# d3sm0/gym_pomdp

Measured on AMD Instinct MI355X. Metric: env steps/sec (whole node), RockSample(7,8) batch=2^20, 1/2/4/8 MI355X, higher is better.
Workload: dtype int32

## Files before the change

gym_pomdp_amd/csrc/envs/rock.hip.h:

```cpp
#pragma once
#include "../envs_common.hip.h"

namespace pomdp {

template <int W, bool STOCH = false>
struct RockEnv {
    using Params = pomdp_rock_params;
    using Reward = int32_t;
    using S = typename std::conditional<W == 1, uint32_t, uint64_t>::type;
    static constexpr int WORDS = W;
    static constexpr const char *NAME = STOCH ? (W == 1 ? "StochasticRockEnv<1>" : "StochasticRockEnv<2>") : (W == 1 ? "RockEnv<1>" : "RockEnv<2>");
    static constexpr bool POOLED_LPT2 = !STOCH;
    static constexpr bool QUAD_STEP = true;
    static constexpr bool HAS_ROCKS = true;
    static constexpr bool POOLED_ANY_LPT = !STOCH;
    static constexpr bool STOCHASTIC = STOCH;
    static constexpr bool QUAD_TAB = true;
    struct Shared {
        uint2 thr[32];
        int8_t grid[256];
        uint8_t rxy[16];
        uint16_t rpos[16];
        uint32_t dir_y[16];
        uint32_t dir_x[16];
// ... 43 lines not shown
        sh.dir_x[tid] = left | (right << 16);
        sh.row[tid] = same;
    }

    static __device__ __forceinline__ void load(State &st, const uint32_t *state, int64_t n, uint32_t i)
    {
        st.s = ld_stream(state + i);
        if (W == 2) st.s |= (S)((uint64_t)ld_stream(state + n + i) << 32);
    }
    static __device__ __forceinline__ void store(const State &st, uint32_t *state, int64_t n, uint32_t i, bool)
    {
        st_stream(state + i, (uint32_t)st.s);
        if (W == 2) st_stream(state + n + i, (uint32_t)((uint64_t)st.s >> 32));
    }

    static __device__ __forceinline__ uint32_t elem(const uint4 &w, uint32_t e) { return e == 0 ? w.x : e == 1 ? w.y : e == 2 ? w.z : w.w; }

    template <class LowWord>
    static __device__ __forceinline__ bool k53_le(uint32_t H, uint32_t th, uint32_t tl, LowWord lo)
    {
        const uint32_t kh = H >> 5;
        bool r = kh < th;
        if (kh == th) r = (lo() >> 6) <= tl;
        return r;
    }
    static __device__ __forceinline__ uint32_t rock_code_hi(uint32_t H)
    {
        const uint32_t kh = H >> 5;
        return kh > HALF_HI ? 2u : (kh < HALF_HI ? 0u : 3u);
    }
    static __device__ __forceinline__ uint32_t rock_code_lo(uint32_t L) { return (L >> 6) ? 2u : 1u; }
    template <bool AUTO = false>
    static __device__ __forceinline__ uint4 reset_block(const RngKey &key, uint32_t lane, uint32_t j2)
    {
        const uint32_t c3 = AUTO ? (((uint32_t)POMDP_STREAM_STEP << 24) | (SENSOR_BLOCK + j2)) : (((uint32_t)POMDP_STREAM_RESET << 24) | j2);
        return philox4x32_10(lane >> 2, key.t_lo, key.t_hi, c3, key.k0, key.k1);
    }
    template <bool AUTO>
    static __device__ __forceinline__ uint32_t reset_codes(const RngKey &key, uint32_t lane, int K)
    {
        return reset_codes<AUTO>(elem(reset_block<AUTO>(key, lane, 0u), lane & 3u), key, lane, K);
    }
    template <bool AUTO>
    static __device__ __forceinline__ uint32_t reset_codes(uint32_t w, const RngKey &key, uint32_t lane, int K)
    {
        uint32_t codes = w & 0xAAAAAAAAu;
        if (__popc(w) <= 6) reset_ties<AUTO>(w, key, lane, K, codes, 0);
        return codes & (K >= 16 ? 0xFFFFFFFFu : ((1u << (2 * K)) - 1u));
    }
    template <bool AUTO>
    static __device__ __forceinline__ void reset_ties(uint32_t w, const RngKey &key, uint32_t lane, int K, uint32_t &word, int base)
    {
        bool have_lo = false;
        uint32_t l = 0;
        for (int j = 0; j < K; ++j) {
            const uint32_t rot = (uint32_t)(2 * j + 2) & 31u;
            if (rock_code_hi(__builtin_rotateright32(w, rot)) != 3u) continue;
            if (!have_lo) {
                uint32_t lane_ = lane;
                asm volatile("" : "+v"(lane_));
                l = elem(reset_block<AUTO>(rare_key(key), lane_, 1u), lane & 3u);
                have_lo = true;
            }
            const uint32_t c = rock_code_lo(__builtin_rotateright32(l, rot));
            word = (word & ~(3u << (base + 2 * j))) | (c << (base + 2 * j));
        }
    }
    static __device__ __forceinline__ uint4 quad_block(const RngKey &key, uint32_t lane, uint32_t j2)
    {
        return philox4x32_10(lane >> 2, key.t_lo, key.t_hi, ((uint32_t)POMDP_STREAM_STEP << 24) | j2, key.k0, key.k1);
    }

    static __device__ __forceinline__ void reset_codes4(const uint32_t (&R)[4], const RngKey &key, uint32_t first, int K,
                                                        uint32_t (&codes)[4])
    {
        const uint32_t exist = K >= 16 ? 0xFFFFFFFFu : ((1u << (2 * K)) - 1u);
#pragma unroll
        for (int e = 0; e < 4; ++e) codes[e] = R[e] & 0xAAAAAAAAu & exist;
        if (min(min(__popc(R[0]), __popc(R[1])), min(__popc(R[2]), __popc(R[3]))) <= 6) {
#pragma unroll
            for (int e = 0; e < 4; ++e) codes[e] = reset_codes<true>(R[e], key, first + (uint32_t)e, K);
        }
    }
    template <int N, bool ROT>
    static __device__ __forceinline__ void fresh_states(const uint32_t (&R)[N], const RngKey &key, uint32_t first, int K,
                                                        uint32_t start, uint32_t (&fresh)[N])
    {
        const uint32_t exist = K >= 16 ? 0xFFFFFFFFu : ((1u << (2 * K)) - 1u);
        auto word = [&](uint32_t codes) { return ROT ? (codes | start) : (start | (codes << 8)); };
        int fewest = __popc(R[0]);
#pragma unroll
        for (int e = 0; e < N; ++e) { fresh[e] = word(R[e] & (0xAAAAAAAAu & exist)); fewest = min(fewest, (int)__popc(R[e])); }
        if (fewest <= 6) {
#pragma unroll
            for (int e = 0; e < N; ++e)
                if (__popc(R[e]) <= 6) reset_ties<true>(R[e], key, first + (uint32_t)e, K, fresh[e], ROT ? 0 : 8);
        }
    }
    static __device__ __forceinline__ int reset(const Shared &, const Params &p, State &st, const RngKey &key,
                                                uint32_t lane)
    {
        const uint64_t s = (uint32_t)p.start_x | ((uint32_t)p.start_y << 4);
        st.s = (S)(s | ((uint64_t)reset_codes<false>(key, lane, p.num_rocks) << 8));
        return 0;
    }
    static __device__ __forceinline__ int reset_ob(const Params &, const State &) { return 0; }

    static __device__ __forceinline__ void reset_where(const Shared &, const Params &p, State &st, bool fresh,
                                                       const RngKey &key, uint32_t lane)
    {
        if (!__any(fresh)) return;
        const uint32_t codes = reset_codes<true>(key, lane, p.num_rocks);
        if (fresh) st.s = (S)((uint64_t)((uint32_t)p.start_x | ((uint32_t)p.start_y << 4)) | ((uint64_t)codes << 8));
    }
    static __device__ __forceinline__ void reset_where_chain(const Shared &sh, const Params &p, State &st, bool fresh,
                                                             const RngKey &key, uint32_t lane, const RngKey &akey,
                                                             uint32_t n_actions, int &next_action)
    {
        reset_where_chain_default<RockEnv>(sh, p, st, fresh, key, lane, akey, n_actions, next_action);
    }
    static __device__ __forceinline__ S fresh_state(const Params &p, uint32_t w, const RngKey &key, uint32_t lane)
    {
        return (S)((uint64_t)((uint32_t)p.start_x | ((uint32_t)p.start_y << 4)) | ((uint64_t)reset_codes<true>(w, key, lane, p.num_rocks) << 8));
    }

    static __device__ __forceinline__ int legal_count(const Shared &sh, const Params &p, const State &st, uint32_t &pre,
                                                      int &n_pre, uint32_t &alive)
    {
        const S s = st.s;
        const int x = (int)(s & 15u), y = (int)((s >> 4) & 15u), K = p.num_rocks;
        pre = 1u; n_pre = 1;
        if (y + 1 < p.size) { pre |= 0u << (3 * n_pre); ++n_pre; }
        if (y - 1 >= 0) { pre |= 2u << (3 * n_pre); ++n_pre; }
        if (x - 1 >= 0) { pre |= 3u << (3 * n_pre); ++n_pre; }
        const int id = sh.grid[x * 16 + y];
        if (id >= 0 && id < K && ((uint32_t)(s >> (8 + 2 * (id & 15))) & 3u) != 1u) { pre |= 4u << (3 * n_pre); ++n_pre; }
        const uint64_t r = (uint64_t)s >> 8;
        const uint64_t even = 0x5555555555555555ull;
        const uint64_t spread = ~(r & ~(r >> 1)) & even & ((1ull << (2 * K)) - 1ull);
        alive = (uint32_t)spread;
        return n_pre + __popc(alive);
    }
    struct Legal { uint32_t pre, alive; int n_pre, count; };
    static __device__ __forceinline__ Legal legal_set(const Shared &sh, const Params &p, const State &st)
    {
        Legal L;
        L.count = legal_count(sh, p, st, L.pre, L.n_pre, L.alive);
        return L;
    }
    static __device__ __forceinline__ int legal_pick(const Shared &sh, const Legal &L, int idx)
    {
        if (idx < L.n_pre) return (int)((L.pre >> (3 * idx)) & 7u);
        const int j = nth_set_bit<2>(L.alive, idx - L.n_pre) >> 1;
        const uint32_t rxy = sh.rxy[j & 15];
        return 5 + sh.grid[(rxy & 15u) * 16 + (rxy >> 4)];
    }
    static __device__ __forceinline__ int legal_nth(const Shared &sh, const Params &p, const State &st, int idx)
    {
        return legal_pick(sh, legal_set(sh, p, st), idx);
    }
    static __device__ __forceinline__ int legal_count(const Shared &sh, const Params &p, const State &st)
    {
        uint32_t pre, alive; int n_pre;
        return legal_count(sh, p, st, pre, n_pre, alive);
    }

    static __device__ __forceinline__ bool check_ok(int measured, int count, double pv)
    {
        return measured < 5 && abs(count) < 2 && 0 < pv && pv < 1;
    }
    static __device__ __forceinline__ void belief_update(const Shared &sh, const Params &p, const State &st, int a, int ob,
                                                         const pomdp_rock_belief &b, int64_t n, uint32_t i, uint32_t &ck)
    {
        const S s = st.s;
        const int x = (int)(s & 15u), y = (int)((s >> 4) & 15u), r = (a - 5) & 15;
        const uint32_t rxy = sh.rxy[r];
// ... 48 lines not shown
        const bool north = (am & dy & 0xFFFFu) != 0, south = (am & (dy >> 16)) != 0;
        const bool west = (same & dx & 0xFFFFu) != 0, east = (same & (dx >> 16)) != 0;
        uint32_t m = (alive & ck) << 5;
        if (y + 1 < p.size && north) m |= 1u << 0;
        if (east) m |= 1u << 1;
        if (y - 1 >= 0 && south) m |= 1u << 2;
        if (x - 1 >= 0 && west) m |= 1u << 3;
        return m;
    }

    static __device__ __forceinline__ int select_target(const Shared &sh, const Params &p, const State &st,
                                                        const pomdp_rock_belief &b, int64_t n, uint32_t i)
    {
        const S s = st.s;
        const int x = (int)(s & 15u), y = (int)((s >> 4) & 15u), K = p.num_rocks;
        int best = 4 * p.size * p.size, best_rock = -1;
        for (int j = 0; j < K; ++j) {
            if (((uint32_t)(s >> (8 + 2 * j)) & 3u) == 1u || b.count[(int64_t)j * n + i] < 0) continue;
            const uint32_t rxy = sh.rxy[j];
            const int dx = x - (int)(rxy & 15u), dy = y - (int)(rxy >> 4), d2 = dx * dx + dy * dy;
            if (d2 < best) { best = d2; best_rock = j; }
        }
        return best_rock;
    }

    static __device__ __forceinline__ double compute_prob(const Shared &sh, const Params &p, const State &st, int a, int ob)
    {
        if (a <= 4) return ob == 0 ? 1.0 : 0.0;
        const S s = st.s;
        const int x = (int)(s & 15u), y = (int)((s >> 4) & 15u), r = (a - 5) & 15;
        const uint32_t rxy = sh.rxy[r];
        const double eff = p.eff[abs(x - (int)(rxy & 15u)) + abs(y - (int)(rxy >> 4))];
        const uint32_t code = (uint32_t)(s >> (8 + 2 * r)) & 3u;
        if ((ob == 2 && code == 2u) || (ob == 1 && code == 0u)) return eff;
        return 1 - eff;
    }

    template <class RT>
    static __device__ __forceinline__ void step_pre(const Shared &sh, const Params &p, State &st, int a, RT &rew,
                                                    int &done, Aux &aux)
    {
        const S s = st.s;
        const uint32_t x = (uint32_t)s & 15u, y = ((uint32_t)s >> 4) & 15u;
        const uint32_t size = (uint32_t)p.size, K = (uint32_t)p.num_rocks;
        const int r = (a - 5) & 15;
        const uint32_t rp = sh.rpos[r];
        const uint32_t d = __builtin_amdgcn_sad_u8(x | (y << 8), rp, 0u);
        aux.th = sh.thr[d].x;
        aux.r = (uint8_t)r;
        aux.good = ((uint32_t)(s >> (8 + 2 * r)) & 3u) == 2u;
        aux.want = a > 4;
        const int penalty = STOCH ? 0 : -100;
        const int id = sh.grid[x * 16 + y];
        const int sh_ = 8 + 2 * (id & 15);
        const uint32_t code = (uint32_t)(s >> sh_) & 3u;
        const bool sample_ok = ((uint32_t)id < K) & (code != 1u);
        const uint32_t a2 = (uint32_t)a << 1;
        const uint32_t nx = x + (uint32_t)__builtin_amdgcn_sbfe(0xC4, a2, 2u), ny = y + (uint32_t)__builtin_amdgcn_sbfe(0x31, a2, 2u);
        const bool inside = max(nx, ny) < size;
        const bool is_move = a < 4, is_sample = a == 4, east = a == 1;
        const bool moved = is_move & inside, left = is_move & !inside, sampled = is_sample & sample_ok,
                   missed = is_sample & !sample_ok;
        const uint32_t d_move = ((uint32_t)s & 0xFFu) ^ (nx | (ny << 4));
        const S d_sample = (S)(code ^ 1u) << sh_;
        st.s = s ^ (moved ? (S)d_move : (sampled ? d_sample : (S)0));
        const bool good_rock = code == 2u;
        int rw = ((left & east) | (sampled & good_rock)) ? 10 : 0;
        rw = (sampled & !good_rock) ? -10 : rw;
        rw = ((left & !east) | missed) ? penalty : rw;
        rew = rw;
        if (STOCH) done = left & east;
        else done = left | missed;
    }
    static __device__ __forceinline__ uint32_t thr_lo_of(const Shared &sh, const State &st, int r)
    {
        const uint32_t x = (uint32_t)st.s & 15u, y = ((uint32_t)st.s >> 4) & 15u;
        return sh.thr[__builtin_amdgcn_sad_u8(x | (y << 8), sh.rpos[r & 15], 0u)].y;
    }
    static constexpr int TAB_ACTIONS = W == 1 ? 17 : 21;

    static constexpr uint32_t REC_LUT_LO = 0x0A0A9CF6u, REC_LUT_HI = 0x00000000u;
    using TabEntry = typename std::conditional<W == 1, uint2, uint32_t>::type;
    struct RecTab { TabEntry e[TAB_ACTIONS][256]; };
    static __device__ __forceinline__ uint32_t rec_f(uint32_t off, int c, uint32_t ob_mask, uint32_t oc)
    {
        const uint32_t rbyte = (((uint64_t)REC_LUT_HI << 32 | REC_LUT_LO) >> (8u * oc)) & 0xFFu;
        return off | (((uint32_t)c & 3u) << 5) | (ob_mask << 8) | (rbyte << 16) | ((oc & 1u) << 24);
    }
    static constexpr uint32_t ROT_POS = 24u;
    template <bool ROT = false>
    static __device__ __forceinline__ void build_rec_tab(RecTab &tab, const Shared &sh, const Params &p, int pos)
    {
        static_assert(!ROT || W == 1, "the rotated layout is the one-state-word loops'");
        constexpr uint32_t POS0 = ROT ? ROT_POS : 0u, ROCK0 = ROT ? 0u : 8u;
        const uint32_t x = (uint32_t)pos & 15u, y = (uint32_t)pos >> 4, size = (uint32_t)p.size, K = (uint32_t)p.num_rocks;
        const int id = sh.grid[x * 16 + y];
        const uint32_t NOTHING = 6u << 28, PENALTY = (STOCH ? 6u : 1u) << 28, EXIT_EAST = 3u << 28;
        const uint32_t NO_TIE = 1u << 27;
        for (int a = 0; a < 5 + (int)K && a < TAB_ACTIONS; ++a) {
            uint32_t e, f;
            if (a < 4) {
                const uint32_t nx = x + (uint32_t)((a == 1) - (a == 3)), ny = y + (uint32_t)((a == 0) - (a == 2));
                const bool inside = max(nx, ny) < size;
                e = inside ? (((uint32_t)pos ^ (nx | (ny << 4))) | NOTHING) : (a == 1 ? EXIT_EAST : PENALTY);
                e |= NO_TIE;
                f = rec_f(POS0 + ((a & 1) ? 0u : 4u), inside ? (a < 2 ? 1 : -1) : 0, 0u, e >> 28 & 7u);
            } else if (a == 4) {
                const bool rock = (uint32_t)id < K;
                e = (rock ? ((8u + 2u * (uint32_t)id) | 0x80000000u) : 0u) | PENALTY | NO_TIE;
                f = rec_f(rock ? ROCK0 + 2u * (uint32_t)id : 0u, 0, 0u, e >> 28 & 7u);
            } else {
                e = sh.thr[__builtin_amdgcn_sad_u8(x | (y << 8), sh.rpos[a - 5], 0u) & 31u].x | NOTHING;
                f = rec_f(ROCK0 + 2u * (uint32_t)(a - 5), 0, 3u, 6u);
            }
            if constexpr (W == 1) tab.e[a][pos] = make_uint2(e, f);
            else tab.e[a][pos] = e;
        }
    }
    template <bool ROT = false>
    static __device__ __forceinline__ uint2 rec_lookup(const RecTab &tab, uint32_t s, uint32_t a)
    {
        if constexpr (ROT) {
            const uint32_t off = __builtin_amdgcn_alignbit(a, s, ROT_POS - 3u) & ~7u;
            return *reinterpret_cast<const uint2 *>(reinterpret_cast<const char *>(&tab.e[0][0]) + off);
        } else return tab.e[a][s & 0xFFu];
    }
    static __device__ __forceinline__ uint32_t rec_kh(uint32_t H) { return __builtin_amdgcn_alignbit(12u, H, 5u); }
    template <bool ROT = false>
    static __device__ __forceinline__ uint32_t rec_thr_lo(const Shared &sh, uint32_t s, uint32_t a, uint32_t f)
    {
        if constexpr (ROT) return thr_lo_of(sh, State{(S)(s >> ROT_POS)}, (int)((f & 31u) >> 1));
        else return thr_lo_of(sh, State{(S)s}, (int)a - 5);
    }
    static __device__ __forceinline__ void rec_finish(const uint2 ef, uint32_t &s, uint32_t a, bool correct, uint32_t fresh, uint32_t &rec)
    {
        const uint32_t e = ef.x, f = ef.y;
        const uint32_t q = __builtin_amdgcn_ubfe(s, f, 2u);
        const bool ok = ((int32_t)e < 0) & (q != 1u);
        const uint32_t keep = ((q == 2u) == correct) ? 0xFFFFFE00u : 0xFFFFFD00u;
        const uint32_t rfb = (f & keep) | a;
        const uint32_t rok = 0x00F60004u - q * 0x00760000u;
        rec = ok ? rok : rfb;
        const int c = ok ? 1 - (int)q : __builtin_amdgcn_sbfe((int)f, 5u, 2u);
        const uint32_t moved = s + ((uint32_t)c << (f & 31u));
        s = rec >= (1u << 24) ? fresh : moved;
    }
    template <class LowWord>
    static __device__ __forceinline__ void step_rec(const Shared &sh, const RecTab &tab, S &s, uint32_t a, uint32_t H, S fresh,
                                                    uint32_t &rec, LowWord lo)
    {
        const uint32_t s_lo = (uint32_t)s, s_hi = W == 2 ? (uint32_t)((uint64_t)s >> 32) : 0u;
        if constexpr (W == 1) {
            const uint2 ef = rec_lookup(tab, s_lo, a);
            const uint32_t kh = rec_kh(H);
            bool correct = kh < ef.x;
            if (kh == ef.x) correct = (lo() >> 6) <= rec_thr_lo(sh, s_lo, a, ef.y);
            uint32_t sn = s_lo;
            rec_finish(ef, sn, a, correct, (uint32_t)fresh, rec);
            s = (S)sn;
        } else {
            const uint32_t e = tab.e[a][s_lo & 0xFFu];
            const bool up_s = (e & 32u) != 0u;
            const uint32_t code = __builtin_amdgcn_ubfe(up_s ? s_hi : s_lo, e, 2u);
            const bool ok = ((int32_t)e < 0) & (code != 1u);
            const uint32_t collect = (code ^ 1u) << (e & 31u);
            const uint32_t move = (a < 4u ? e : 0u) & 0xFFu;
            const uint32_t d_lo = (ok & !up_s) ? collect : move, d_hi = (ok & up_s) ? collect : 0u;
            const uint32_t oc = ok ? code : __builtin_amdgcn_ubfe(e, 28u, 3u);
            const uint32_t rbyte = __builtin_amdgcn_perm(REC_LUT_HI, REC_LUT_LO, (oc << 16) | 0x0C000C0Cu);
            const uint32_t done = oc & 1u;
            const uint32_t gi = 2u * a - 1u;
            const bool good = __builtin_amdgcn_ubfe((gi & 32u) ? s_hi : s_lo, gi, 1u) != 0u;
            const uint32_t kh = __builtin_amdgcn_alignbit(12u, H, 5u);
            bool correct = kh < e;
            if (a > 4u && kh == e) correct = (lo() >> 6) <= thr_lo_of(sh, State{s}, (int)a - 5);
            const uint32_t ob = a > 4u ? ((good == correct) ? 2u << 8 : 1u << 8) : 0u;
            rec = rbyte | (done << 24) | ob | a;
            s = done ? fresh : (S)(((uint64_t)(s_hi ^ d_hi) << 32) | (s_lo ^ d_lo));
        }
    }

    template <class LowWord>
    static __device__ __forceinline__ int sensor_ob(const Shared &sh, const State &st, const Aux &aux, uint32_t H, LowWord lo)
    {
        const uint32_t kh = H >> 5;
        bool correct = kh < aux.th;
        if (kh == aux.th) correct = (lo() >> 6) <= thr_lo_of(sh, st, aux.r);
        return aux.want ? ((aux.good == correct) ? 2 : 1) : 0;
    }

    static constexpr bool QUAD_SENSOR = !STOCH;
    template <class RT>
    static __device__ __forceinline__ void step_with_H(const Shared &sh, const Params &p, State &st, int a, const RngKey &key,
                                                       uint32_t lane, uint32_t H, int &ob, RT &rew, int &done)
    {
        Aux aux;
        step_pre(sh, p, st, a, rew, done, aux);
        ob = sensor_ob(sh, st, aux, H, [&]() { return elem(quad_block(key, lane, 1u), lane & 3u); });
    }

    template <class RT>
    static __device__ __forceinline__ void step(const Shared &sh, const Params &p, State &st, int a,
                                                const RngKey &key, uint32_t lane, int &ob, RT &rew, int &done)
    {
        const uint32_t e = lane & 3u;
        if (STOCH) {
            const uint4 g = quad_block(key, lane, 0u);
            const bool act = k53_le(elem(g, e), (uint32_t)(p.act_thr >> 26), (uint32_t)p.act_thr & LO_MASK,
                                    [&]() { return elem(quad_block(key, lane, 1u), e); }) != (p.act_gt != 0);
            State nx = st;
            Aux aux; RT r2; int d2;
            step_pre(sh, p, nx, a, r2, d2, aux);
            const uint4 h = quad_block(key, lane, 2u);
            const int o2 = sensor_ob(sh, nx, aux, elem(h, e), [&]() { return elem(quad_block(key, lane, 3u), e); });
            if (act) { st = nx; rew = r2; done = d2; ob = o2; }
            else { rew = 0; done = 0; ob = 0; }
            return;
        }
        Aux aux;
        step_pre(sh, p, st, a, rew, done, aux);
        const uint4 h = quad_block(key, lane, 0u);
        ob = sensor_ob(sh, st, aux, elem(h, e), [&]() { return elem(quad_block(key, lane, 1u), e); });
    }
};

}
```

gym_pomdp_amd/csrc/fused_impl.hip.h:

```cpp
#pragma once
#include "kernels_common.hip.h"

namespace pomdp {

template <class L, class Pol, int LPT = 4, bool SROW = false>
struct FusedCtx {
    uint32_t l0, glane0;
    uint64_t t0;
    typename lanes_out<L, LPT, SROW>::type out;
    typename lanes_policy<Pol, LPT>::type pol;
    uint32_t n_bad;
    __device__ __forceinline__ FusedCtx(int32_t *action, int32_t *ob, void *reward, uint8_t *done, int64_t rec, uint32_t lane0,
                                        const RngKey &key0, const RngKey &akey0, uint32_t n_act, int k_steps, const TapeRef &tape)
        : l0(blockIdx.x * (uint32_t)(LPT * BLOCK) + (uint32_t)LPT * threadIdx.x), glane0(lane0 + l0),
          t0(((uint64_t)key0.t_hi << 32) | key0.t_lo), out(action, ob, reward, done, rec, l0),
          pol(tape, l0, glane0, key0, akey0, n_act, k_steps), n_bad(0) {}
    __device__ __forceinline__ void first(int gen_first, int (&a_cur)[LPT])
    {
        if constexpr (LPT == 4) {
            const u32x4 a4 = out.first(pol, gen_first);
#pragma unroll
            for (int j = 0; j < 4; ++j) a_cur[j] = (int)a4[j];
        } else {
            uint32_t a2[LPT];
// ... 172 lines not shown
            else if constexpr (quad_policy && quad_words_of<Env>::value == 3) {
                if (sj == 0) { step_quarter(s); if constexpr (POLICY_WITH_STEP) policy_quarter(s); }
                auto pick = [&](const uint4 &q) { return pick4(q); };
                Env::step_words(sh, p, st[j], valid[j] ? a_cur[j] : 0, key, glane[j], pick(nq0), pick(nq1), pick(nq2), o[j], r[j], d[j]);
            }
            else Fin::lane_step(sh, p, st[j], valid[j] ? a_cur[j] : 0, key, glane[j], o[j], r[j], d[j], aux[j]);
            if (!live[j]) { r[j] = 0; d[j] = was_done[j]; }
            fresh[j] = live[j] && d[j] && auto_reset;
            a_next[j] = 0;
        }
        if constexpr (quad_policy) {
            if constexpr (!TAPE && !POLICY_WITH_STEP) { if (sj == 0) policy_quarter(s); }
            if constexpr (REC) {
            } else if constexpr (Env::QUAD_SENSOR) {
                const uint32_t rword = pick4(rq);
                st[0].s = fresh[0] ? Env::fresh_state(p, rword, key, glane[0]) : st[0].s;
            } else if constexpr (quad_word_env<Env>::value) {
                Env::fresh_w(sh, p, st[0], fresh[0], key, glane[0], pick4(sq));
            } else {
                Fin::resets_only(sh, p, st, fresh, key, glane);
            }
            const uint32_t word = pick4(aq);
            if constexpr (!TAPE) a_next[0] = (int)__umulhi(word, (uint32_t)n_act);
        } else {
            Fin::run(sh, p, st, fresh, key, glane, akey, (uint32_t)n_act, a_next, aux, o);
        }
#pragma unroll
        for (int j = 0; j < LPT; ++j) {
            if (!live[j]) { o[j] = 0; st[j] = before[j]; }
            if (in_range[j]) out.put_next_action(rel[j], a_next[j]);
            ever_fresh[j] |= fresh[j];
            if (in_range[j]) {
                uint32_t rcode = 0;
                if constexpr (L::CODES && !REC) rcode = Env::reward_code(r[j]);
                if constexpr (REC && L::CODES) out.put_record(j, rel[j], recv[j]);
                else out.put(j, rel[j], a_cur[j], o[j], r[j], rcode, d[j]);
                if (!valid[j] && !was_done[j] && err) atomicAdd(err, 1u);
            }
            if constexpr (TAPE4) a_next[j] = (int)tq[(std::decay_t<decltype(sj_)>::value + 1) & 3];
            else if constexpr (TAPE) a_next[j] = (int)col.nxt;
            a_cur[j] = a_next[j];
            was_done[j] = auto_reset ? false : (d[j] != 0);
        }
        out.next_row();
        if constexpr (Fin::LOOP_BARRIER && !quad_policy) __syncthreads();
    };
    if constexpr (UNROLL4 && UNROLL4_TAIL) {
        #pragma unroll 1
        for (int seg = 0, s = 0; seg < 4; ++seg) {
            const int seg_end = prio.template segment<4>(seg);
            #pragma unroll 1
            for (; s + 4 <= seg_end; s += 4) {
                step_body(s, std::integral_constant<int, 0>{});
                step_body(s + 1, std::integral_constant<int, 1>{});
                step_body(s + 2, std::integral_constant<int, 2>{});
                step_body(s + 3, std::integral_constant<int, 3>{});
            }
            #pragma unroll 1
            for (; s < seg_end; ++s) step_body(s, s & 3);
        }
    } else if constexpr (UNROLL4) {
        #pragma unroll 1
        for (int seg = 0, s = 0; seg < 4; ++seg)
        for (const int seg_end = prio.template segment<4>(seg); s < seg_end; s += 4) {
            step_body(s, std::integral_constant<int, 0>{});
            if (s + 1 < seg_end) {
                step_body(s + 1, std::integral_constant<int, 1>{});
                if (s + 2 < seg_end) {
                    step_body(s + 2, std::integral_constant<int, 2>{});
                    if (s + 3 < seg_end) step_body(s + 3, std::integral_constant<int, 3>{});
                }
            }
        }
    } else {
        #pragma unroll 1
        for (int seg = 0, s = 0; seg < 4; ++seg)
        for (const int seg_end = prio.segment(seg); s < seg_end; ++s) step_body(s, s & 3);
    }
#pragma unroll
    for (int j = 0; j < LPT; ++j)
        if (in_range[j]) { Env::store(st[j], state_w, n, rel[j], ever_fresh[j]); out.finish(j, rel[j], k_steps); }
}

template <class Env, class L = Columns, class Pol = SyntheticQuad, int LPT = 4>
__global__ __launch_bounds__(BLOCK) void steps_quad_kernel(uint32_t *__restrict__ state, int32_t *__restrict__ action,
                                                           int32_t *__restrict__ ob, int32_t *__restrict__ reward,
                                                           uint8_t *__restrict__ done, int64_t n, RngKey key0, uint32_t lane0,
                                                           RngKey akey0, int k_steps, int64_t rec, int gen_first,
                                                           const typename Env::Params p, TapeRef tape)
{
    static_assert(LPT == 4 || LPT == 2, "a quad or half a quad per thread");
    constexpr int W = Env::WORDS;
    constexpr bool ROT = W == 1;
    using S = typename Env::S;
    __shared__ typename Env::Shared sh;
    __shared__ typename Env::RecTab tab;
    const uint32_t n_act = (uint32_t)Env::n_actions(p);
    constexpr bool AHEAD2 = Pol::TAPE && LPT == 4;
    using PolT = typename std::conditional<AHEAD2, TapeQuadAhead, Pol>::type;
    FusedCtx<L, PolT, LPT, true> cx(action, ob, reward, done, rec, lane0, key0, akey0, n_act, k_steps, tape);
    const uint32_t l0 = cx.l0, glane0 = cx.glane0;
    const uint32_t e0 = LPT == 4 ? 0u : (glane0 & 2u);
    typename Env::State st[LPT];
    int a_cur[LPT];
    uint32_t sp0 = 0, sp1 = 0, gp0 = 0, gp1 = 0;
    {
        uint32_t s_lo[LPT], s_hi[LPT];
        if constexpr (LPT == 4) {
            const u32x4 lo = ld_stream4(state + l0);
            u32x4 hi = {0, 0, 0, 0};
            if (W == 2) hi = ld_stream4(state + n + l0);
#pragma unroll
            for (int j = 0; j < 4; ++j) { s_lo[j] = lo[j]; s_hi[j] = hi[j]; }
        } else {
            const u32x2 lo = ld_stream2(state + l0);
            u32x2 hi = {0, 0};
            if (W == 2) hi = ld_stream2(state + n + l0);
#pragma unroll
            for (int j = 0; j < 2; ++j) { s_lo[j] = lo[j]; s_hi[j] = hi[j]; }
        }
        cx.first(gen_first, a_cur);
#pragma unroll
        for (int j = 0; j < LPT; ++j) {
            if constexpr (ROT) st[j].s = __builtin_amdgcn_alignbit(s_lo[j], s_lo[j], 8u);
            else st[j].s = (S)((uint64_t)s_lo[j] | ((uint64_t)s_hi[j] << 32));
        }
    }
    Env::stage(sh, p, (int)threadIdx.x);
    __syncthreads();
    Env::template build_rec_tab<ROT>(tab, sh, p, (int)threadIdx.x);
    __syncthreads();
    const int K = p.num_rocks;
    const uint32_t start = (uint32_t)p.start_x | ((uint32_t)p.start_y << 4);
    uint32_t start_rot = start << (ROT ? Env::ROT_POS : 0u);
    if constexpr (ROT) asm volatile("" : "+v"(start_rot));
    const LoopPrio prio(k_steps);
    constexpr uint32_t SENSOR_BLOCK = Env::SENSOR_BLOCK;
    const PhiloxFixed sensor_fx = philox_fixed(glane0 >> 2, ((uint32_t)POMDP_STREAM_STEP << 24) | SENSOR_BLOCK, key0.k1);
    const PhiloxFixed gate_fx = philox_fixed(glane0 >> 2, (uint32_t)POMDP_STREAM_STEP << 24, key0.k1);
    auto step_body = [&](const int s, const auto par_) __attribute__((always_inline)) {
        constexpr int PAR = decltype(par_)::value;
        const RngKey key = cx.key(key0, s);
        uint32_t H[LPT], G[LPT];
        if constexpr (LPT == 4) {
            const uint4 sw = philox4x32_10_fixed(sensor_fx, key.t_lo, key.t_hi, key.k0, key.k1);
            H[0] = sw.x; H[1] = sw.y; H[2] = sw.z; H[3] = sw.w;
        } else {
            pair_shared(s, e0 != 0u, [&](int sb) { return Env::quad_block(cx.key(key0, sb), glane0, SENSOR_BLOCK); }, H, sp0, sp1);
        }
        uint32_t a_next[LPT];
        if constexpr (AHEAD2) cx.pol.template begin_par<PAR>(s, a_next);
        else cx.pol.begin(s, a_next);
        bool acts[LPT];
#pragma unroll
        for (int j = 0; j < LPT; ++j) acts[j] = true;
        if constexpr (Env::STOCHASTIC) {
            if constexpr (LPT == 4) {
                const uint4 gw = philox4x32_10_fixed(gate_fx, key.t_lo, key.t_hi, key.k0, key.k1);
                G[0] = gw.x; G[1] = gw.y; G[2] = gw.z; G[3] = gw.w;
            } else {
                pair_shared(s, e0 != 0u, [&](int sb) { return Env::quad_block(cx.key(key0, sb), glane0, 0u); }, G, gp0, gp1);
            }
#pragma unroll
            for (int j = 0; j < LPT; ++j)
                acts[j] = Env::k53_le(G[j], (uint32_t)(p.act_thr >> 26), (uint32_t)p.act_thr & Env::LO_MASK,
                                      [&]() { return Env::elem(Env::quad_block(key, glane0, 1u), e0 + (uint32_t)j); }) != (p.act_gt != 0);
        }
        uint32_t rec[LPT], a_taken[LPT];
#pragma unroll
        for (int j = 0; j < LPT; ++j) a_taken[j] = (uint32_t)a_cur[j];
        bool valid[LPT];
#pragma unroll
        for (int j = 0; j < LPT; ++j) valid[j] = !Pol::TAPE || a_taken[j] < n_act;
        auto low_word = [&](int j) __attribute__((always_inline)) {
            return Env::elem(Env::quad_block(rare_key(key), glane0 + (uint32_t)j, SENSOR_BLOCK + 1u), e0 + (uint32_t)j);
        };
        if constexpr (ROT) {
            uint32_t fresh[LPT], kh[LPT], sn[LPT];
            uint2 ef[LPT];
            bool correct[LPT], tie[LPT], any_tie = false;
            Env::template fresh_states<LPT, true>(H, key, glane0, K, start_rot, fresh);
#pragma unroll
            for (int j = 0; j < LPT; ++j) ef[j] = Env::template rec_lookup<true>(tab, st[j].s, valid[j] ? a_taken[j] : 0u);
            if constexpr (LPT == 4) asm volatile("" : "+v"(ef[0].x), "+v"(ef[0].y), "+v"(ef[1].x), "+v"(ef[1].y), "+v"(ef[2].x), "+v"(ef[2].y), "+v"(ef[3].x), "+v"(ef[3].y));
            else asm volatile("" : "+v"(ef[0].x), "+v"(ef[0].y), "+v"(ef[1].x), "+v"(ef[1].y));
#pragma unroll
            for (int j = 0; j < LPT; ++j) {
                kh[j] = Env::rec_kh(H[j]);
                correct[j] = kh[j] < ef[j].x;
                tie[j] = kh[j] == ef[j].x;
                any_tie |= tie[j];
            }
            if (any_tie) {
#pragma unroll
                for (int j = 0; j < LPT; ++j)
                    if (tie[j]) correct[j] = (low_word(j) >> 6) <= Env::template rec_thr_lo<true>(sh, st[j].s, a_taken[j], ef[j].y);
            }
#pragma unroll
            for (int j = 0; j < LPT; ++j) {
                sn[j] = st[j].s;
                Env::rec_finish(ef[j], sn[j], valid[j] ? a_taken[j] : 0u, correct[j], fresh[j], rec[j]);
            }
#pragma unroll
            for (int j = 0; j < LPT; ++j) {
                if constexpr (Env::STOCHASTIC) {
                    sn[j] = acts[j] ? sn[j] : st[j].s;
                    rec[j] = acts[j] ? rec[j] : a_taken[j];
                }
                if constexpr (Pol::TAPE) {
                    sn[j] = valid[j] ? sn[j] : st[j].s;
                    rec[j] = valid[j] ? rec[j] : a_taken[j];
                    cx.n_bad += (uint32_t)!valid[j];
                }
                st[j].s = sn[j];
            }
        } else {
            uint32_t codes[LPT];
            if constexpr (LPT == 4) Env::reset_codes4(H, key, glane0, K, codes);
            else {
#pragma unroll
                for (int j = 0; j < LPT; ++j) codes[j] = Env::template reset_codes<true>(H[j], key, glane0 + (uint32_t)j, K);
            }
#pragma unroll
            for (int j = 0; j < LPT; ++j) {
                S sj = st[j].s;
                Env::step_rec(sh, tab, sj, valid[j] ? a_taken[j] : 0u, H[j], (S)((uint64_t)start | ((uint64_t)codes[j] << 8)), rec[j],
                              [&]() { return low_word(j); });
                if constexpr (Env::STOCHASTIC) {
                    sj = acts[j] ? sj : st[j].s;
                    rec[j] = acts[j] ? rec[j] : a_taken[j];
                }
                if constexpr (Pol::TAPE) {
                    sj = valid[j] ? sj : st[j].s;
                    rec[j] = valid[j] ? rec[j] : a_taken[j];
                    cx.n_bad += (uint32_t)!valid[j];
                }
                st[j].s = sj;
            }
        }
        cx.out.put_records(rec, a_next);
        if constexpr (AHEAD2) {
            cx.pol.template end_par<PAR>(s, a_next);
#pragma unroll
            for (int j = 0; j < LPT; ++j) a_cur[j] = (int)a_next[j];
        } else cx.advance(s, a_next, a_cur);
    };
    if constexpr (AHEAD2) {
        wait_loads();
        _Pragma("unroll 1") for (int seg = 0, s = 0; seg < 4; ++seg)
            for (const int seg_end = prio.template segment<2>(seg); s < seg_end; s += 2) {
                step_body(s, std::integral_constant<int, 0>{});
                if (s + 1 < seg_end) step_body(s + 1, std::integral_constant<int, 1>{});
            }
    } else {
        POMDP_FUSED_STEP_LOOP(prio, s) step_body(s, std::integral_constant<int, 0>{});
    }
    cx.finish(k_steps);
    uint32_t w_lo[LPT];
#pragma unroll
    for (int j = 0; j < LPT; ++j) w_lo[j] = ROT ? __builtin_amdgcn_alignbit((uint32_t)st[j].s, (uint32_t)st[j].s, 24u) : (uint32_t)st[j].s;
    if constexpr (LPT == 4) {
        st_stream4(state + l0, w_lo[0], w_lo[1], w_lo[2], w_lo[3]);
        if (W == 2)
            st_stream4(state + n + l0, (uint32_t)((uint64_t)st[0].s >> 32), (uint32_t)((uint64_t)st[1].s >> 32),
                       (uint32_t)((uint64_t)st[2].s >> 32), (uint32_t)((uint64_t)st[3].s >> 32));
    } else {
        st_stream2(state + l0, w_lo[0], w_lo[1]);
        if (W == 2) st_stream2(state + n + l0, (uint32_t)((uint64_t)st[0].s >> 32), (uint32_t)((uint64_t)st[1].s >> 32));
    }
}

template <bool TAB, class L = Columns, class Pol = SyntheticQuad, int LPT = 4>
__global__ __launch_bounds__(BLOCK) void tag_steps_quad_kernel(uint32_t *__restrict__ state, int32_t *__restrict__ action,
                                                               int32_t *__restrict__ ob, float *__restrict__ reward,
                                                               uint8_t *__restrict__ done, int64_t n, RngKey key0,
                                                               uint32_t lane0, RngKey akey0, int k_steps, int64_t rec,
                                                               int gen_first, const TagEnv::Params p, TapeRef tape)
{
    using Env = TagEnv;
    static_assert(LPT == 4 || LPT == 2, "a quad or half a quad per thread");
    __shared__ Env::Shared sh;
    __shared__ typename std::conditional<TAB, Env::StepTab, NoTab>::type tab;
    const uint32_t n_act = (uint32_t)Env::n_actions(p);
    FusedCtx<L, Pol, LPT> cx(action, ob, reward, done, rec, lane0, key0, akey0, n_act, k_steps, tape);
    const uint32_t l0 = cx.l0, glane0 = cx.glane0;
    const uint32_t e0 = LPT == 4 ? 0u : (glane0 & 2u);
    Env::State st[LPT];
    int a_cur[LPT];
    uint32_t sp0 = 0, sp1 = 0;
    {
        if constexpr (LPT == 4) {
            const u32x4 s4 = ld_stream4(state + l0);
            cx.first(gen_first, a_cur);
#pragma unroll
            for (int j = 0; j < 4; ++j) st[j].w = s4[j];
        } else {
            const u32x2 s2 = ld_stream2(state + l0);
            cx.first(gen_first, a_cur);
#pragma unroll
            for (int j = 0; j < 2; ++j) st[j].w = s2[j];
        }
    }
    Env::stage(sh, p, (int)threadIdx.x);
    __syncthreads();
    if constexpr (TAB) {
        Env::build_tab(tab, sh, p, (int)threadIdx.x);
        __syncthreads();
    }
    const LoopPrio prio(k_steps);
    POMDP_FUSED_STEP_LOOP(prio, s) {
        const RngKey key = cx.key(key0, s);
        uint32_t a_next[LPT];
        cx.pol.begin(s, a_next);
        int o[LPT], d[LPT];
        float r[LPT];
        uint32_t a_taken[LPT], W[LPT];
#pragma unroll
        for (int j = 0; j < LPT; ++j) a_taken[j] = (uint32_t)a_cur[j];
        if constexpr (LPT == 4) {
            const uint4 qw = Env::quad_block(key, glane0, 0u);
            W[0] = qw.x; W[1] = qw.y; W[2] = qw.z; W[3] = qw.w;
        } else {
            pair_shared(s, e0 != 0u, [&](int sb) { return Env::quad_block(cx.key(key0, sb), glane0, 0u); }, W, sp0, sp1);
        }
#pragma unroll
        for (int j = 0; j < LPT; ++j) {
            Env::Flight f;
            const bool valid = !Pol::TAPE || a_taken[j] < n_act;
            const Env::State before = st[j];
            const int a = valid ? a_cur[j] : 0;
            if constexpr (TAB) Env::step_one_opponent_tab(tab, st[j], a, o[j], r[j], d[j], f);
            else Env::step_one_opponent_pre(sh, p, st[j], a, o[j], r[j], d[j], f);
            const uint32_t lane = glane0 + (uint32_t)j;
            if constexpr (Pol::TAPE) { if (!valid) { f.need = false; o[j] = 0; r[j] = 0.f; d[j] = 0; cx.n_bad++; } }
            Env::flee_word(sh, p, st[j], f, W[j], [&]() { return Env::elem(Env::quad_block(key, lane, 1u), e0 + (uint32_t)j); });
            if (d[j]) Env::auto_reset_word(p, st[j], W[j], key, lane);
            if constexpr (Pol::TAPE) st[j] = valid ? st[j] : before;
        }
        uint32_t o4[LPT], r4[LPT], d4[LPT], rc[LPT];
#pragma unroll
        for (int j = 0; j < LPT; ++j) {
            o4[j] = (uint32_t)o[j]; r4[j] = __float_as_uint(r[j]); d4[j] = (uint32_t)d[j];
            rc[j] = 0;
            if constexpr (L::CODES) rc[j] = Env::reward_code(r[j]);
        }
        cx.out.put(a_taken, a_next, o4, r4, rc, d4);
        cx.advance(s, a_next, a_cur);
    }
    cx.finish(k_steps);
    if constexpr (LPT == 4) st_stream4(state + l0, st[0].w, st[1].w, st[2].w, st[3].w);
    else st_stream2(state + l0, st[0].w, st[1].w);
}
// ... 521 lines not shown
#define POMDP_LAUNCH_PAIR(...)                                                                                           \
    do {                                                                                                                 \
        const dim3 pgrid((unsigned)(n / (2 * BLOCK)));                                                                   \
        if (taped) hipLaunchKernelGGL((__VA_ARGS__, TapeQuad, 2>), pgrid, dim3(BLOCK), 0, (hipStream_t)stream, POMDP_QUAD_ARGS); \
        else hipLaunchKernelGGL((__VA_ARGS__, SyntheticQuad, 2>), pgrid, dim3(BLOCK), 0, (hipStream_t)stream, POMDP_QUAD_ARGS); \
    } while (0)
    if constexpr (std::is_same<Env, TagEnv>::value) {
        if constexpr (pair_sink<L>::value) {
            if (quad_ok && n >= TAG_PAIR_MIN_LANES && n <= TAG_PAIR_MAX_LANES && p.num_opponents == 1 && k >= 16 && TagEnv::tab_ok(p)) {
                char pname[40];
                snprintf(pname, sizeof pname, "%s, 2", lname);
                note_fused("tag_steps_quad_kernel", "true", pname);
                POMDP_LAUNCH_PAIR(tag_steps_quad_kernel<true, L);
                launched = true;
            }
        }
        if (!launched && quad_ok && n >= QUAD_MIN_TAG && p.num_opponents == 1) {
            if (k >= 16 && TagEnv::tab_ok(p)) {
                note_fused("tag_steps_quad_kernel", "true", lname);
                POMDP_LAUNCH_QUAD(tag_steps_quad_kernel<true, L);
            } else {
                note_fused("tag_steps_quad_kernel", "false", lname);
                POMDP_LAUNCH_QUAD(tag_steps_quad_kernel<false, L);
            }
            launched = true;
        }
    }
    if constexpr (has_next<Env>::value) {
        if constexpr (pair_sink<L>::value) {
            if (quad_ok && n >= BS_PAIR_MIN_LANES && n <= BS_PAIR_MAX_LANES && k <= 256) {
                char pname[40];
                snprintf(pname, sizeof pname, "%s, 2", lname);
                note_fused("battleship_steps_quad_kernel", Env::NAME, pname);
                const dim3 pgrid((unsigned)(n / (2 * BLOCK)));
                if (taped) hipLaunchKernelGGL((battleship_steps_quad_kernel<Env::WORDS / 3, L, TapeQuad, 2, true>), pgrid, dim3(BLOCK), 0, (hipStream_t)stream, POMDP_QUAD_ARGS);
                else hipLaunchKernelGGL((battleship_steps_quad_kernel<Env::WORDS / 3, L, SyntheticQuad, 2, true>), pgrid, dim3(BLOCK), 0, (hipStream_t)stream, POMDP_QUAD_ARGS);
                launched = true;
            }
        }
        if (!launched && quad_ok && n >= QUAD_MIN_BATTLESHIP && k <= 256) {
            note_fused("battleship_steps_quad_kernel", Env::NAME, lname);
            if (n * (Env::WORDS / 3) <= BS_VIS_LDS_MAX_LANES * 4) {
                if constexpr (!std::is_same<L, Columns>::value) {
                    if (taped) hipLaunchKernelGGL((battleship_steps_quad_kernel<Env::WORDS / 3, L, TapeQuad, 4, true>), qgrid, dim3(BLOCK), 0, (hipStream_t)stream, POMDP_QUAD_ARGS);
                }
                if constexpr (!std::is_same<L, ColumnsNoAct>::value) {
                    if (!taped) hipLaunchKernelGGL((battleship_steps_quad_kernel<Env::WORDS / 3, L, SyntheticQuad, 4, true>), qgrid, dim3(BLOCK), 0, (hipStream_t)stream, POMDP_QUAD_ARGS);
                }
            } else POMDP_LAUNCH_QUAD(battleship_steps_quad_kernel<Env::WORDS / 3, L);
            launched = true;
        }
    }
    if constexpr (std::is_same<Env, NetworkEnv>::value) {
        if (quad_ok && n >= QUAD_MIN_NETWORK) {
            const bool small = p.n_machines <= 10 && (p.fail_thr >> 37) != 0 && (p.fail_nb_thr >> 37) != 0;
            snprintf(variant, sizeof variant, "%d, %s, %s%s", small ? 2 : (p.n_machines + 7) / 8, L::NAME, small ? "true" : "false", taped ? ", Tape" : "");
            note_fused("network_steps_quad_kernel", variant, "");
            if (small) {
                POMDP_LAUNCH_QUAD(network_steps_quad_kernel<2, L, true);
            } else
            switch ((p.n_machines + 7) / 8) {
            case 1: POMDP_LAUNCH_QUAD(network_steps_quad_kernel<1, L, false); break;
            case 2: POMDP_LAUNCH_QUAD(network_steps_quad_kernel<2, L, false); break;
            case 3: POMDP_LAUNCH_QUAD(network_steps_quad_kernel<3, L, false); break;
            default: POMDP_LAUNCH_QUAD(network_steps_quad_kernel<4, L, false); break;
            }
            launched = true;
        }
    }
    if constexpr (quad_fused<Env>::value) {
        if (quad_ok && n >= QUAD_MIN_GENERIC) {
            note_fused("steps_quad_generic_kernel", Env::NAME, lname);
            POMDP_LAUNCH_QUAD(steps_quad_generic_kernel<Env, L);
            launched = true;
        }
    }
    if constexpr (quad_tab<Env>::value) {
        if constexpr (pair_sink<L>::value && !RETS) {
            if (quad_ok && n >= (Env::STOCHASTIC ? STOCHROCK_PAIR_MIN_LANES : ROCK_PAIR_MIN_LANES) &&
                n <= (Env::STOCHASTIC ? STOCHROCK_PAIR_MAX_LANES : ROCK_PAIR_MAX_LANES) && k >= 16 && p.num_rocks + 5 <= Env::TAB_ACTIONS) {
                char pname[40];
                snprintf(pname, sizeof pname, "%s, 2", lname);
                note_fused("steps_quad_kernel", Env::NAME, pname);
                const dim3 pgrid((unsigned)(n / (2 * BLOCK)));
                if (taped) hipLaunchKernelGGL((steps_quad_kernel<Env, L, TapeQuad, 2>), pgrid, dim3(BLOCK), 0, (hipStream_t)stream, POMDP_QUAD_ARGS);
                else hipLaunchKernelGGL((steps_quad_kernel<Env, L, SyntheticQuad, 2>), pgrid, dim3(BLOCK), 0, (hipStream_t)stream, POMDP_QUAD_ARGS);
                launched = true;
            }
        }
        if (!launched && quad_ok && n >= (Env::STOCHASTIC ? QUAD_MIN_STOCHROCK : QUAD_MIN_ROCK) && k >= 16 && p.num_rocks + 5 <= Env::TAB_ACTIONS) {
            note_fused("steps_quad_kernel", Env::NAME, lname);
            POMDP_LAUNCH_QUAD(steps_quad_kernel<Env, L);
            launched = true;
        }
    }
    if (taped) {
        if constexpr (!std::is_same<L, Columns>::value) {
            if constexpr (quad_policy_of<Finisher<Env, 1, true>>::value) {
                if (!launched && (flags & POMDP_AUTO_RESET) && n % BLOCK == 0) {
                    bool tab = false;
                    if constexpr (quad_tab<Env>::value && Env::QUAD_SENSOR) tab = k >= 16 && p.num_rocks + 5 <= Env::TAB_ACTIONS;
                    snprintf(variant, sizeof variant, ", 1, true, %s%s", tab ? "true" : "false", lname);
                    note_fused("steps_kernel", Env::NAME, variant);
                    if constexpr (quad_tab<Env>::value && Env::QUAD_SENSOR) {
                        if (tab) hipLaunchKernelGGL((steps_kernel<Env, 1, true, true, L, true>), grid, dim3(BLOCK), 0, (hipStream_t)stream, state, action, ob,
                                                    reward, done, err, n, make_key(seed, t), lane0, kflags, make_key(action_seed, t + 1), k, rec, p, tape);
                    }
                    if (!tab) hipLaunchKernelGGL((steps_kernel<Env, 1, true, false, L, true>), grid, dim3(BLOCK), 0, (hipStream_t)stream, state, action, ob,
                                                 reward, done, err, n, make_key(seed, t), lane0, kflags, make_key(action_seed, t + 1), k, rec, p, tape);
                    launched = true;
                }
            }
            if (!launched) {
                snprintf(variant, sizeof variant, ", 1, false%s%s", COLS ? "" : ", false", lname);
                note_fused("steps_kernel", Env::NAME, variant);
                hipLaunchKernelGGL((steps_kernel<Env, 1, false, false, L, true>), grid, dim3(BLOCK), 0, (hipStream_t)stream, state, action, ob,
                                   reward, done, err, n, make_key(seed, t), lane0, kflags, make_key(action_seed, t + 1), k, rec, p, tape);
            }
        }
        return (int)hipGetLastError();
    }
    if constexpr (!std::is_same<L, ColumnsNoAct>::value) {
    if constexpr (Env::POOLED_ANY_LPT && Env::WORDS == 1) {
        if (!launched && lpt2 && (flags & POMDP_AUTO_RESET) && n % (4 * BLOCK) == 0 && n >= (1 << 20)) {
            POMDP_LAUNCH_STEPS(4, true, qgrid);
            launched = true;
        }
    }
    if constexpr (Env::POOLED_LPT2) {
        if (!launched && lpt2) {
            if (simple) POMDP_LAUNCH_STEPS(2, true, grid); else POMDP_LAUNCH_STEPS(2, false, grid);
            launched = true;
        }
    }
    if constexpr (quad_tab<Env>::value && Env::QUAD_SENSOR) {
        if (!launched && simple && k >= 16 && p.num_rocks + 5 <= Env::TAB_ACTIONS) {
            snprintf(variant, sizeof variant, ", 1, true, true%s", lname);
            note_fused("steps_kernel", Env::NAME, variant);
            hipLaunchKernelGGL((steps_kernel<Env, 1, true, true, L>), grid, dim3(BLOCK), 0, (hipStream_t)stream, state, action, ob, reward,
                               done, err, n, make_key(seed, t), lane0, kflags, make_key(action_seed, t + 1), k, rec, p, tape);
            launched = true;
        }
    }
    if (!launched) { if (simple) POMDP_LAUNCH_STEPS(1, true, grid); else POMDP_LAUNCH_STEPS(1, false, grid); }
    }
#undef POMDP_LAUNCH_STEPS
#undef POMDP_LAUNCH_QUAD
#undef POMDP_QUAD_ARGS
    return (int)hipGetLastError();
}

template <class Env>
int launch_steps_fused(const typename Env::Params &p, uint32_t *state, int32_t *action, int32_t *ob,
                       typename Env::Reward *reward, uint8_t *done, uint32_t *err, int64_t n, uint64_t seed,
                       uint64_t action_seed, uint32_t lane0, uint64_t t, int k, int flags, int64_t rec, bool gen_first,
                       int layout, TapeRef tape, void *stream)
{
#define POMDP_FUSED_L(L_) launch_steps_fused_l<Env, L_>(p, state, action, ob, reward, done, err, n, seed, action_seed, lane0, t, k, flags, rec, gen_first, tape, stream)
    switch (layout) {
    case POMDP_LAYOUT_COLUMNS: return tape.base ? POMDP_FUSED_L(ColumnsNoAct) : POMDP_FUSED_L(Columns);
    case POMDP_LAYOUT_BLOCKED: return POMDP_FUSED_L(Blocked);
    case POMDP_LAYOUT_PACKED: return POMDP_FUSED_L(Packed);
    case POMDP_LAYOUT_NARROW: return POMDP_FUSED_L(Narrow);
    case LAYOUT_RETURNS: return POMDP_FUSED_L(Returns<Env>);
    default: return POMDP_E_BADARG;
    }
#undef POMDP_FUSED_L
}

}
```

Measured before the change: 907.2 billion.

## Compare raw RNG word to prescaled sensor threshold and use numeric reset gate

The sensor-check table now stores a pre-shifted threshold word, so the common path compares the raw random word H against it directly. The exact low-word check only runs when H falls within a small span above the threshold, and the rock flag moves into the f word. The reset-tie gate for up to 8 rocks becomes a numeric min-compare against a bound instead of popcounts, and a separate popc kernel instantiation is dispatched when there are more rocks. The aim is fewer ALU ops per step in the hot quad loop, at the cost of a second kernel instantiation and a wider near-tie branch.

Result: faster. 964.2 billion, median of 6 (+6.3%).

```diff
diff --git a/gym_pomdp_amd/csrc/envs/rock.hip.h b/gym_pomdp_amd/csrc/envs/rock.hip.h
--- a/gym_pomdp_amd/csrc/envs/rock.hip.h
+++ b/gym_pomdp_amd/csrc/envs/rock.hip.h
@@ -149,16 +149,29 @@
             for (int e = 0; e < 4; ++e) codes[e] = reset_codes<true>(R[e], key, first + (uint32_t)e, K);
         }
     }
-    template <int N, bool ROT>
+    static constexpr int RESET_NUMERIC_K = 8;
+    static __device__ __forceinline__ uint32_t reset_tie_bound(int K) { return 1u << (2 * min(K, RESET_NUMERIC_K) + 5); }
+    template <int N, bool ROT, bool NUMERIC>
     static __device__ __forceinline__ void fresh_states(const uint32_t (&R)[N], const RngKey &key, uint32_t first, int K,
-                                                        uint32_t start, uint32_t (&fresh)[N])
+                                                        uint32_t start, uint32_t bound, uint32_t (&fresh)[N])
     {
         const uint32_t exist = K >= 16 ? 0xFFFFFFFFu : ((1u << (2 * K)) - 1u);
         auto word = [&](uint32_t codes) { return ROT ? (codes | start) : (start | (codes << 8)); };
-        int fewest = __popc(R[0]);
 #pragma unroll
-        for (int e = 0; e < N; ++e) { fresh[e] = word(R[e] & (0xAAAAAAAAu & exist)); fewest = min(fewest, (int)__popc(R[e])); }
-        if (fewest <= 6) {
+        for (int e = 0; e < N; ++e) fresh[e] = word(R[e] & (0xAAAAAAAAu & exist));
+        bool look;
+        if constexpr (NUMERIC) {
+            uint32_t least = R[0];
+#pragma unroll
+            for (int e = 1; e < N; ++e) least = min(least, R[e]);
+            look = least < bound;
+        } else {
+            int fewest = __popc(R[0]);
+#pragma unroll
+            for (int e = 1; e < N; ++e) fewest = min(fewest, (int)__popc(R[e]));
+            look = fewest <= 6;
+        }
+        if (look) {
 #pragma unroll
             for (int e = 0; e < N; ++e)
                 if (__popc(R[e]) <= 6) reset_ties<true>(R[e], key, first + (uint32_t)e, K, fresh[e], ROT ? 0 : 8);
@@ -373,6 +386,9 @@
     static constexpr uint32_t REC_LUT_LO = 0x0A0A9CF6u, REC_LUT_HI = 0x00000000u;
     using TabEntry = typename std::conditional<W == 1, uint2, uint32_t>::type;
     struct RecTab { TabEntry e[TAB_ACTIONS][256]; };
+    static constexpr uint32_t REC_ROCK = 1u << 31;
+    static constexpr uint32_t TIE_SPAN = 32u;
+    static __device__ __forceinline__ uint32_t rec_thr_word(uint32_t T) { return T >= (1u << 27) ? 0xFFFFFFFFu : T << 5; }
     static __device__ __forceinline__ uint32_t rec_f(uint32_t off, int c, uint32_t ob_mask, uint32_t oc)
     {
         const uint32_t rbyte = (((uint64_t)REC_LUT_HI << 32 | REC_LUT_LO) >> (8u * oc)) & 0xFFu;
@@ -404,7 +420,7 @@
                 e = sh.thr[__builtin_amdgcn_sad_u8(x | (y << 8), sh.rpos[a - 5], 0u) & 31u].x | NOTHING;
                 f = rec_f(ROCK0 + 2u * (uint32_t)(a - 5), 0, 3u, 6u);
             }
-            if constexpr (W == 1) tab.e[a][pos] = make_uint2(e, f);
+            if constexpr (W == 1) tab.e[a][pos] = make_uint2(a > 4 ? rec_thr_word(e & ~NOTHING) : 0xFFFFFFFFu, f | (a == 4 ? e & REC_ROCK : 0u));
             else tab.e[a][pos] = e;
         }
     }
@@ -416,19 +432,22 @@
             return *reinterpret_cast<const uint2 *>(reinterpret_cast<const char *>(&tab.e[0][0]) + off);
         } else return tab.e[a][s & 0xFFu];
     }
-    static __device__ __forceinline__ uint32_t rec_kh(uint32_t H) { return __builtin_amdgcn_alignbit(12u, H, 5u); }
-    template <bool ROT = false>
-    static __device__ __forceinline__ uint32_t rec_thr_lo(const Shared &sh, uint32_t s, uint32_t a, uint32_t f)
-    {
-        if constexpr (ROT) return thr_lo_of(sh, State{(S)(s >> ROT_POS)}, (int)((f & 31u) >> 1));
-        else return thr_lo_of(sh, State{(S)s}, (int)a - 5);
+    template <bool ROT = false, class LowWord>
+    static __device__ __forceinline__ bool rec_sensor_exact(const Shared &sh, uint32_t s, uint32_t f, uint32_t H, LowWord lo)
+    {
+        const uint32_t pos = ROT ? s >> ROT_POS : s, r = (((f & 31u) - (ROT ? 0u : 8u)) >> 1) & 15u;
+        const uint2 t = sh.thr[__builtin_amdgcn_sad_u8((pos & 15u) | ((pos & 0xF0u) << 4), sh.rpos[r], 0u) & 31u];
+        const uint32_t kh = H >> 5;
+        uint32_t kl = lo() >> 6;
+        asm volatile("" : "+v"(kl));
+        return kh == t.x ? kl <= t.y : kh < t.x;
     }
     static __device__ __forceinline__ void rec_finish(const uint2 ef, uint32_t &s, uint32_t a, bool correct, uint32_t fresh, uint32_t &rec)
     {
-        const uint32_t e = ef.x, f = ef.y;
+        const uint32_t f = ef.y;
         const uint32_t q = __builtin_amdgcn_ubfe(s, f, 2u);
-        const bool ok = ((int32_t)e < 0) & (q != 1u);
-        const uint32_t keep = ((q == 2u) == correct) ? 0xFFFFFE00u : 0xFFFFFD00u;
+        const bool ok = ((int32_t)f < 0) & (q != 1u);
+        const uint32_t keep = ((q == 2u) == correct) ? 0x7FFFFE00u : 0x7FFFFD00u;
         const uint32_t rfb = (f & keep) | a;
         const uint32_t rok = 0x00F60004u - q * 0x00760000u;
         rec = ok ? rok : rfb;
@@ -443,9 +462,8 @@
         const uint32_t s_lo = (uint32_t)s, s_hi = W == 2 ? (uint32_t)((uint64_t)s >> 32) : 0u;
         if constexpr (W == 1) {
             const uint2 ef = rec_lookup(tab, s_lo, a);
-            const uint32_t kh = rec_kh(H);
-            bool correct = kh < ef.x;
-            if (kh == ef.x) correct = (lo() >> 6) <= rec_thr_lo(sh, s_lo, a, ef.y);
+            bool correct = H < ef.x;
+            if (H - ef.x < TIE_SPAN) correct = rec_sensor_exact(sh, s_lo, ef.y, H, lo);
             uint32_t sn = s_lo;
             rec_finish(ef, sn, a, correct, (uint32_t)fresh, rec);
             s = (S)sn;
diff --git a/gym_pomdp_amd/csrc/fused_impl.hip.h b/gym_pomdp_amd/csrc/fused_impl.hip.h
--- a/gym_pomdp_amd/csrc/fused_impl.hip.h
+++ b/gym_pomdp_amd/csrc/fused_impl.hip.h
@@ -278,12 +278,12 @@
         if (in_range[j]) { Env::store(st[j], state_w, n, rel[j], ever_fresh[j]); out.finish(j, rel[j], k_steps); }
 }
 
-template <class Env, class L = Columns, class Pol = SyntheticQuad, int LPT = 4>
-__global__ __launch_bounds__(BLOCK) void steps_quad_kernel(uint32_t *__restrict__ state, int32_t *__restrict__ action,
-                                                           int32_t *__restrict__ ob, int32_t *__restrict__ reward,
-                                                           uint8_t *__restrict__ done, int64_t n, RngKey key0, uint32_t lane0,
-                                                           RngKey akey0, int k_steps, int64_t rec, int gen_first,
-                                                           const typename Env::Params p, TapeRef tape)
+template <class Env, class L, class Pol, int LPT, bool NUMERIC>
+__device__ __forceinline__ void steps_quad_body(uint32_t *__restrict__ state, int32_t *__restrict__ action,
+                                                int32_t *__restrict__ ob, int32_t *__restrict__ reward,
+                                                uint8_t *__restrict__ done, int64_t n, RngKey key0, uint32_t lane0,
+                                                RngKey akey0, int k_steps, int64_t rec, int gen_first,
+                                                const typename Env::Params &p, TapeRef tape)
 {
     static_assert(LPT == 4 || LPT == 2, "a quad or half a quad per thread");
     constexpr int W = Env::WORDS;
@@ -334,6 +334,8 @@
     constexpr uint32_t SENSOR_BLOCK = Env::SENSOR_BLOCK;
     const PhiloxFixed sensor_fx = philox_fixed(glane0 >> 2, ((uint32_t)POMDP_STREAM_STEP << 24) | SENSOR_BLOCK, key0.k1);
     const PhiloxFixed gate_fx = philox_fixed(glane0 >> 2, (uint32_t)POMDP_STREAM_STEP << 24, key0.k1);
+    uint32_t tie_bound = 0;
+    if constexpr (ROT && NUMERIC) { tie_bound = Env::reset_tie_bound(K); asm volatile("" : "+s"(tie_bound)); }
     auto step_body = [&](const int s, const auto par_) __attribute__((always_inline)) {
         constexpr int PAR = decltype(par_)::value;
         const RngKey key = cx.key(key0, s);
@@ -372,25 +374,32 @@
             return Env::elem(Env::quad_block(rare_key(key), glane0 + (uint32_t)j, SENSOR_BLOCK + 1u), e0 + (uint32_t)j);
         };
         if constexpr (ROT) {
-            uint32_t fresh[LPT], kh[LPT], sn[LPT];
+            uint32_t fresh[LPT], sn[LPT];
             uint2 ef[LPT];
-            bool correct[LPT], tie[LPT], any_tie = false;
-            Env::template fresh_states<LPT, true>(H, key, glane0, K, start_rot, fresh);
+            Env::template fresh_states<LPT, true, NUMERIC>(H, key, glane0, K, start_rot, tie_bound, fresh);
 #pragma unroll
             for (int j = 0; j < LPT; ++j) ef[j] = Env::template rec_lookup<true>(tab, st[j].s, valid[j] ? a_taken[j] : 0u);
-            if constexpr (LPT == 4) asm volatile("" : "+v"(ef[0].x), "+v"(ef[0].y), "+v"(ef[1].x), "+v"(ef[1].y), "+v"(ef[2].x), "+v"(ef[2].y), "+v"(ef[3].x), "+v"(ef[3].y));
-            else asm volatile("" : "+v"(ef[0].x), "+v"(ef[0].y), "+v"(ef[1].x), "+v"(ef[1].y));
-#pragma unroll
-            for (int j = 0; j < LPT; ++j) {
-                kh[j] = Env::rec_kh(H[j]);
-                correct[j] = kh[j] < ef[j].x;
-                tie[j] = kh[j] == ef[j].x;
-                any_tie |= tie[j];
-            }
-            if (any_tie) {
+            {
+                uint64_t w[LPT];
+#pragma unroll
+                for (int j = 0; j < LPT; ++j) w[j] = (uint64_t)ef[j].x | ((uint64_t)ef[j].y << 32);
+                if constexpr (LPT == 4) asm volatile("" : "+v"(w[0]), "+v"(w[1]), "+v"(w[2]), "+v"(w[3]));
+                else asm volatile("" : "+v"(w[0]), "+v"(w[1]));
+#pragma unroll
+                for (int j = 0; j < LPT; ++j) ef[j] = make_uint2((uint32_t)w[j], (uint32_t)(w[j] >> 32));
+            }
+            uint32_t near[LPT];
+            bool correct[LPT];
+#pragma unroll
+            for (int j = 0; j < LPT; ++j) correct[j] = __builtin_sub_overflow(H[j], ef[j].x, &near[j]);
+            uint32_t nearest = near[0];
+#pragma unroll
+            for (int j = 1; j < LPT; ++j) nearest = min(nearest, near[j]);
+            if (nearest < Env::TIE_SPAN) {
 #pragma unroll
                 for (int j = 0; j < LPT; ++j)
-                    if (tie[j]) correct[j] = (low_word(j) >> 6) <= Env::template rec_thr_lo<true>(sh, st[j].s, a_taken[j], ef[j].y);
+                    if (near[j] < Env::TIE_SPAN)
+                        correct[j] = Env::template rec_sensor_exact<true>(sh, st[j].s, ef[j].y, H[j], [&]() { return low_word(j); });
             }
 #pragma unroll
             for (int j = 0; j < LPT; ++j) {
@@ -464,6 +473,25 @@
         st_stream2(state + l0, w_lo[0], w_lo[1]);
         if (W == 2) st_stream2(state + n + l0, (uint32_t)((uint64_t)st[0].s >> 32), (uint32_t)((uint64_t)st[1].s >> 32));
     }
+}
+template <class Env, class L = Columns, class Pol = SyntheticQuad, int LPT = 4>
+__global__ __launch_bounds__(BLOCK) void steps_quad_kernel(uint32_t *__restrict__ state, int32_t *__restrict__ action,
+                                                           int32_t *__restrict__ ob, int32_t *__restrict__ reward,
+                                                           uint8_t *__restrict__ done, int64_t n, RngKey key0, uint32_t lane0,
+                                                           RngKey akey0, int k_steps, int64_t rec, int gen_first,
+                                                           const typename Env::Params p, TapeRef tape)
+{
+    steps_quad_body<Env, L, Pol, LPT, Env::WORDS == 1>(state, action, ob, reward, done, n, key0, lane0, akey0, k_steps, rec, gen_first, p, tape);
+}
+template <class Env, class L = Columns, class Pol = SyntheticQuad, int LPT = 4>
+__global__ __launch_bounds__(BLOCK) void steps_quad_popc_kernel(uint32_t *__restrict__ state, int32_t *__restrict__ action,
+                                                                int32_t *__restrict__ ob, int32_t *__restrict__ reward,
+                                                                uint8_t *__restrict__ done, int64_t n, RngKey key0, uint32_t lane0,
+                                                                RngKey akey0, int k_steps, int64_t rec, int gen_first,
+                                                                const typename Env::Params p, TapeRef tape)
+{
+    static_assert(Env::WORDS == 1, "two state words take reset_codes4");
+    steps_quad_body<Env, L, Pol, LPT, false>(state, action, ob, reward, done, n, key0, lane0, akey0, k_steps, rec, gen_first, p, tape);
 }
 
 template <bool TAB, class L = Columns, class Pol = SyntheticQuad, int LPT = 4>
@@ -1151,15 +1179,19 @@
                 char pname[40];
                 snprintf(pname, sizeof pname, "%s, 2", lname);
                 note_fused("steps_quad_kernel", Env::NAME, pname);
-                const dim3 pgrid((unsigned)(n / (2 * BLOCK)));
-                if (taped) hipLaunchKernelGGL((steps_quad_kernel<Env, L, TapeQuad, 2>), pgrid, dim3(BLOCK), 0, (hipStream_t)stream, POMDP_QUAD_ARGS);
-                else hipLaunchKernelGGL((steps_quad_kernel<Env, L, SyntheticQuad, 2>), pgrid, dim3(BLOCK), 0, (hipStream_t)stream, POMDP_QUAD_ARGS);
+                bool popc = false;
+                if constexpr (Env::WORDS == 1) popc = p.num_rocks > Env::RESET_NUMERIC_K;
+                if constexpr (Env::WORDS == 1) { if (popc) POMDP_LAUNCH_PAIR(steps_quad_popc_kernel<Env, L); }
+                if (!popc) POMDP_LAUNCH_PAIR(steps_quad_kernel<Env, L);
                 launched = true;
             }
         }
         if (!launched && quad_ok && n >= (Env::STOCHASTIC ? QUAD_MIN_STOCHROCK : QUAD_MIN_ROCK) && k >= 16 && p.num_rocks + 5 <= Env::TAB_ACTIONS) {
             note_fused("steps_quad_kernel", Env::NAME, lname);
-            POMDP_LAUNCH_QUAD(steps_quad_kernel<Env, L);
+            bool popc = false;
+            if constexpr (Env::WORDS == 1) popc = p.num_rocks > Env::RESET_NUMERIC_K;
+            if constexpr (Env::WORDS == 1) { if (popc) POMDP_LAUNCH_QUAD(steps_quad_popc_kernel<Env, L); }
+            if (!popc) POMDP_LAUNCH_QUAD(steps_quad_kernel<Env, L);
             launched = true;
         }
     }
```
